# byronknoll/gmix

Hardware: AMD Instinct MI355X
Metric: mixer bits/sec (synthetic 256-input mixer streams, forward+update) (higher is better)
Workload: dtype f32; 1 GPU; configs[1]: synthetic 256-input 1-layer mixer (1 mixer, 2^16-row gate table), random logits, forward+update; n_inputs=256, mixers=1/0/0, streams_per_gpu=4096, total_bits=5486149632, parallelism=streams sharded over 1 GPU(s), no collective on the data path

## Files before the change

gmix_amd/csrc/gmx_capi.cpp:

```cpp
#include <hip/hip_runtime.h>
#include <math.h>
#include <stddef.h>
#include <stdio.h>
#include <stdlib.h>
#include <string.h>
#include <time.h>

#include <algorithm>
#include <atomic>
#include <map>
#include <new>
#include <string>
#include <vector>

#include "../../include/gmxmix.h"
#include "gmx_buildhash.h"
#include "gmx_internal.h"
#include "gmx_mailbox.h"
#include "gmx_ckpt.h"
#include "gmx_ind_ckpt.h"
#include "gmx_match.h"
#include "gmx_match_ckpt.h"
#include "gmx_ctx.h"
#include "gmx_ctx_ckpt.h"
// ... 220 lines not shown
  *dev_out = c.dev[k];
  return GMX_OK;
}
static int count_list_used(GmxCountList& c, hipStream_t st) {
  const int k = (int)((c.seq - 1u) % (unsigned)kStageSlots);
  HIPCHK(hipEventRecord(c.done[k], st));
  c.busy[k] = true;
  return GMX_OK;
}

struct gmx_group {
  int device = 0;
  int S = 0;
  GmxTopoDev topo;
  GmxTopoDev* topo_dev = nullptr;
  uint8_t* banks = nullptr;
  float* latch_out = nullptr;
  hipStream_t stream = nullptr;
  hipEvent_t ev0 = nullptr, ev1 = nullptr;
  unsigned lds_bytes = 0;
  std::vector<uint64_t> steps;
  std::vector<uint8_t> fwd_done;
  struct DecaySlot {
    float* dev = nullptr;
    uint32_t* idx_dev = nullptr;
    float* host = nullptr;
    uint32_t* idx_host = nullptr;
    size_t cap = 0;
    size_t idx_cap = 0;
    hipEvent_t done = nullptr;
    hipEvent_t ready = nullptr;
    bool busy = false;
    uint64_t* st_dev = nullptr;
    uint64_t* st_host = nullptr;
    uint32_t* amb_dev = nullptr;
    uint32_t* amb_host = nullptr;
    float* patch_host = nullptr;
    size_t st_cap = 0;
  } decay[kStageSlots];
  GmxCountList counts;
  hipStream_t copy_stream = nullptr;
  hipStream_t up_stream = nullptr, down_stream = nullptr;
  unsigned run_seq = 0;
  hipEvent_t tm0 = nullptr, tm1 = nullptr;
  gmx_batch* one = nullptr;
  std::vector<gmx_batch*> batches;
  std::vector<struct GmxSession*> sessions;
  std::vector<struct gmx_lockstep*> locksteps;
  bool banks_in_use_by_dead_kernel = false;
  bool use_sessions = true;
  bool mailbox_on_device = true;
  bool force_general = false;
  bool stock_exact = false;
  int stock_staged = -1;
  bool decay_on_host = false;
  bool stock_pairs = false;
  bool register_rows = false;
  int single_variant = 0;
  struct GmxCkptState* ckpt = nullptr;
};

struct gmx_batch {
  gmx_group* g = nullptr;
  int S = 0;
  uint64_t max_bits = 0;
  unsigned flags = 0;
  float* d_pred = nullptr;
  uint32_t* d_mask = nullptr;
  uint32_t* d_ctx = nullptr;
  uint8_t* d_bits = nullptr;
  float* d_p = nullptr;
  float* d_out = nullptr;
  float* d_last = nullptr;
  uint64_t* d_rng = nullptr;
  uint64_t* d_tcount = nullptr;
  float* d_pstate = nullptr;
  uint32_t* d_cstate = nullptr;
  float* h_pred = nullptr;
  uint32_t* h_mask = nullptr;
  uint32_t* h_ctx = nullptr;
  uint8_t* h_bits = nullptr;
  float* h_p = nullptr;
  float* h_out = nullptr;
  float* h_last = nullptr;
  GmxXfer x;
};

struct gmx_lockstep {
  gmx_group* g = nullptr;
  gmx_batch* b = nullptr;
  float* dec_host = nullptr;
  uint8_t* bits_host = nullptr;
  float* dec_dev = nullptr;
  uint32_t* idx_dev = nullptr;
  hipGraph_t g_predict = nullptr, g_learn = nullptr, g_step = nullptr;
  hipGraphExec_t x_predict = nullptr, x_learn = nullptr, x_step = nullptr;
  bool predicted = false;
  bool persistent = false, ps_running = false, ps_dead = false, ps_counted = false;
  hipStream_t ps_stream = nullptr;
  GmxLsDoor* door = nullptr;
  uint32_t* done = nullptr;
  uint32_t* blk_seen = nullptr;
  uint32_t* blk_replay = nullptr;
  uint32_t* relay = nullptr;
  float* live = nullptr;
  uint32_t seq = 0, word = 0, completed = 0;
// ... 458 lines not shown
  const bool wide = g->topo.l0 == 24 && g->topo.l1 == 8 && g->topo.n_skip == 1 && g->topo.has_final &&
                    ((g->topo.n == 256 && g->topo.mx[23].stride == 288) ||
                     (g->topo.n == 90 && g->topo.mx[23].stride == 128 && g->stock_pairs && !g->stock_exact)) &&
                    (mode & GMX_MODE_PREDICT) && !(mode & GMX_MODE_LATCH) && !g->force_general;
  return single ? GMX_K_SINGLE : wide ? GMX_K_WIDE : stock ? GMX_K_STOCK : GMX_K_BANK;
}

static int launch_run(gmx_group* g, gmx_batch* b, int s0, int rec0, int ns, uint64_t T,
                      unsigned mode, float* kernel_ms, const uint64_t* n_list = nullptr) {
  if (T == 0) return GMX_OK;
  for (gmx_lockstep* ls : g->locksteps) ls->predicted = false;
  gmx_group::DecaySlot* dec = nullptr;
  int rc = prepare_decay(g, s0, ns, T, (mode & GMX_MODE_LEARN) ? 1 : 0, &dec);
  if (rc) return rc;
  GmxRunArgs a;
  memset(&a, 0, sizeof a);
  a.banks = g->banks;
  a.pred = b->d_pred;
  a.mask = (b->flags & GMX_BATCH_MASK) ? b->d_mask : nullptr;
  a.ctx = b->d_ctx;
  a.bits = b->d_bits;
  a.decay = dec->dev;
  a.decay_idx = dec->idx_dev;
  a.p_out = b->d_p;
  a.out_all = (b->flags & GMX_BATCH_OUTPUTS) ? b->d_out : nullptr;
  a.out_last = (b->flags & GMX_BATCH_LAST_OUTPUTS) ? b->d_last : nullptr;
  a.latch_out = g->latch_out;
  a.rec_stride = b->max_bits;
  a.T = T;
  if (n_list) {
    int rcl = count_list_stage(g->counts, n_list, ns, g->stream, &a.T_list);
    if (rcl) return rcl;
  }
  a.mode = mode | (g->stock_exact ? GMX_MODE_EXACT : 0u);
  a.stream_base = s0;
  a.rec_base = rec0;
  a.n_streams = ns;
  {
    int rcx = xfer_before_run(b->x, g->stream);
    if (rcx) return rcx;
  }
  if (kernel_ms) HIPCHK(hipEventRecord(g->ev0, g->stream));
  const GmxKernelKind kind = kernel_for(g, mode);
  const bool single = kind == GMX_K_SINGLE, wide = kind == GMX_K_WIDE, stock = kind == GMX_K_STOCK;
  if (a.out_last && (single || wide)) return GMX_ERR_INVALID;
  if (kind == GMX_K_PAIR)
    HIPCHK(gmx_launch_pair_kernel(g->topo_dev, &a, ns, a.mask != nullptr, g->topo.n, g->topo.l0, g->topo.l1, g->stream));
  else if (single)
    HIPCHK(gmx_launch_single_kernel(g->topo_dev, &a, g->topo.n, g->single_variant, g->stream));
  else if (wide)
    HIPCHK(gmx_launch_wide_kernel(g->topo_dev, &a, ns, a.mask != nullptr, g->topo.n, g->stream));
  else if (stock)
    HIPCHK(gmx_launch_stock_kernel(g->topo_dev, &a, ns, GMX_STK_LDS_BYTES(g->topo.lds_misc),
                                   a.mask != nullptr, g->stock_staged, topo_tables_pow2(g->topo), g->stream));
  else
    HIPCHK(gmx_launch_bank_kernel(g->topo_dev, &a, ns, g->lds_bytes, a.mask != nullptr, g->topo.l0,
                                  g->topo.l1, g->topo.n_skip, g->topo.has_final,
                                  g->topo.mx[g->topo.l0 - 1].stride, g->stream));
  HIPCHK(hipEventRecord(dec->done, g->stream));
  dec->busy = true;
  if (n_list) {
    int rcl = count_list_used(g->counts, g->stream);
    if (rcl) return rcl;
  }
  {
    int rcn = batch_note_device_use(b);
    if (rcn) return rcn;
  }
  if (kernel_ms) {
    HIPCHK(hipEventRecord(g->ev1, g->stream));
    HIPCHK(hipEventSynchronize(g->ev1));
    HIPCHK(hipEventElapsedTime(kernel_ms, g->ev0, g->ev1));
  }
  if (mode & GMX_MODE_LEARN)
    for (int i = 0; i < ns; ++i) g->steps[s0 + i] += n_list ? n_list[i] : T;
  return GMX_OK;
}

static void batch_free(gmx_batch* b) {
  if (!b) return;
  if (b->g) {
    (void)hipSetDevice(b->g->device);
    if (b->g->stream) (void)hipStreamSynchronize(b->g->stream);
    if (b->g->up_stream) (void)hipStreamSynchronize(b->g->up_stream);
    if (b->g->down_stream) (void)hipStreamSynchronize(b->g->down_stream);
    auto& v = b->g->batches;
    v.erase(std::remove(v.begin(), v.end(), b), v.end());
  }
  void* dv[] = {b->d_pred, b->d_mask, b->d_ctx, b->d_bits, b->d_p, b->d_out, b->d_last,
                b->d_rng, b->d_tcount, b->d_pstate, b->d_cstate};
  for (void* p : dv)
    if (p) (void)hipFree(p);
  void* hv[] = {b->h_pred, b->h_mask, b->h_ctx, b->h_bits, b->h_p, b->h_out, b->h_last};
  for (void* p : hv)
    if (p) (void)hipHostFree(p);
  xfer_free(b->x);
  delete b;
}

static int batch_alloc(gmx_batch** out, gmx_group* g, int S, uint64_t max_bits, unsigned flags) {
  if (!out || !g || max_bits == 0) return GMX_ERR_INVALID;
  *out = nullptr;
  HIPCHK(hipSetDevice(g->device));
  gmx_batch* b = new (std::nothrow) gmx_batch();
  if (!b) return GMX_ERR_NOMEM;
  b->g = g;
  b->S = S;
// ... 504 lines not shown
  }
  HIPCHK(hipMalloc((void**)&tmp.dev, uniq.size() * T * sizeof(float)));
  int rc = decay_table_on_device(g, tmp, uniq, T);
  if (rc == GMX_OK) {
    if (n_unsettled) *n_unsettled = tmp.amb_host[0];
    std::vector<float> h(uniq.size() * T);
    hipError_t e = hipMemcpyAsync(h.data(), tmp.dev, h.size() * sizeof(float), hipMemcpyDeviceToHost, g->copy_stream);
    if (e == hipSuccess) e = hipStreamSynchronize(g->copy_stream);
    if (e != hipSuccess) rc = hip_fail(e, "gmx_debug_decay_table copy");
    else
      for (int u = 0; u < U; ++u) memcpy(out + (size_t)u * T, h.data() + (size_t)row[u] * T, T * sizeof(float));
  }
  void* dv[] = {tmp.dev, tmp.st_dev, tmp.amb_dev};
  for (void* p : dv)
    if (p) (void)hipFree(p);
  void* hv[] = {tmp.st_host, tmp.amb_host, tmp.patch_host};
  for (void* p : hv)
    if (p) (void)hipHostFree(p);
  return rc;
}

extern "C" int gmx_topology_register_rows_eligible(const gmx_topology* topo) {
  GmxTopoDev td;
  if (build_topology(topo, &td) != GMX_OK) return GMX_ERR_INVALID;
  return topo_register_rows_eligible(td) ? 1 : 0;
}

extern "C" int gmx_group_set_register_rows(gmx_group* g, int on) {
  if (!g || !topo_register_rows_eligible(g->topo)) return GMX_ERR_INVALID;
  g->register_rows = on != 0;
  return GMX_OK;
}

extern "C" int gmx_debug_force_general(gmx_group* g, int on) {
  if (!g) return GMX_ERR_INVALID;
  g->force_general = on != 0;
  return GMX_OK;
}

extern "C" int gmx_debug_kernel_kind(gmx_group* g, unsigned mode) {
  if (!g) return GMX_ERR_INVALID;
  const GmxKernelKind kind = kernel_for(g, mode);
  if (kind != GMX_K_BANK) return (int)kind;
  const GmxTopoDev& t = g->topo;
  return (int)kind + 4 * gmx_bank_kernel_build(t.l0, t.l1, t.n_skip, t.has_final, t.mx[t.l0 - 1].stride);
}

extern "C" int gmx_debug_stock_staged(gmx_group* g, int mode) {
  if (!g || mode < -1 || mode > 1) return GMX_ERR_INVALID;
  g->stock_staged = mode;
  return GMX_OK;
}

extern "C" int gmx_debug_stock_exact(gmx_group* g, int on) {
  if (!g) return GMX_ERR_INVALID;
  int rc = sessions_close(g, true);
  if (rc) return rc;
  g->stock_exact = on != 0;
  return GMX_OK;
}

extern "C" int gmx_debug_use_sessions(gmx_group* g, int on) {
  if (!g) return GMX_ERR_INVALID;
  int rc = sessions_close(g, true);
  if (rc) return rc;
  for (GmxSession* se : g->sessions)
    if (se && se->fwd_live) return GMX_ERR_STATE;
  g->use_sessions = on != 0;
  return GMX_OK;
}

extern "C" int gmx_debug_open_sessions(void) { return g_open_sessions.load(); }

extern "C" int gmx_debug_mailbox_on_device(gmx_group* g, int on, int stream, int* active) {
  if (!g) return GMX_ERR_INVALID;
  if (active) {
    GmxSession* se = (stream >= 0 && stream < (int)g->sessions.size()) ? g->sessions[stream] : nullptr;
    *active = (se && se->mc_on_device) ? 1 : 0;
  }
  if ((on != 0) == g->mailbox_on_device) return GMX_OK;
  int rc = sessions_close(g, true);
  if (rc) return rc;
  for (GmxSession* se : g->sessions)
    if (se && se->fwd_live) return GMX_ERR_STATE;
  sessions_free(g);
  g->mailbox_on_device = on != 0;
  return GMX_OK;
}

extern "C" int gmx_debug_per_bit_latency(gmx_group* g, int stream, int n, int ctx_hold, double* us_per_bit) {
  if (!g || n <= 0 || ctx_hold <= 0 || !us_per_bit) return GMX_ERR_INVALID;
  const GmxTopoDev& t = g->topo;
  std::vector<float> pred(t.n);
  std::vector<uint32_t> ctx(t.m, 0);
  uint64_t x = 0x9E3779B97F4A7C15ull;
  auto rnd = [&x]() { x ^= x << 13; x ^= x >> 7; x ^= x << 17; return x; };
  timespec a, b;
  clock_gettime(CLOCK_MONOTONIC, &a);
  for (int i = 0; i < n; ++i) {
    for (int k = 0; k < t.n; ++k) pred[k] = (float)((int64_t)(rnd() >> 40) - (1 << 23)) * (1.0f / (1 << 21));
    if (i % ctx_hold == 0)
      for (int k = 0; k < t.m; ++k) ctx[k] = (uint32_t)rnd();
    float p;
    int rc = gmx_bank_forward(g, stream, pred.data(), nullptr, -1, ctx.data(), &p, nullptr);
    if (rc) return rc;
    rc = gmx_bank_learn(g, stream, p > 0.5f ? 1 : 0);
// ... 461 lines not shown
```

gmix_amd/csrc/gmx_math.h:

```cpp
#ifndef GMX_MATH_H_
#define GMX_MATH_H_

#include <stdint.h>
#include <string.h>
#ifndef __cplusplus
#include <stdbool.h>
#endif

#if defined(__HIPCC__)
#include <hip/hip_runtime.h>
#define GMX_HD __host__ __device__ __forceinline__
#else
#define GMX_HD static inline
#endif

#if defined(__HIP_DEVICE_COMPILE__)
__device__ __constant__
#endif
static const uint64_t gmx_exp2f_tab[32] = {
    0x3ff0000000000000ull, 0x3fefd9b0d3158574ull, 0x3fefb5586cf9890full, 0x3fef9301d0125b51ull,
    0x3fef72b83c7d517bull, 0x3fef54873168b9aaull, 0x3fef387a6e756238ull, 0x3fef1e9df51fdee1ull,
    0x3fef06fe0a31b715ull, 0x3feef1a7373aa9cbull, 0x3feedea64c123422ull, 0x3feece086061892dull,
    0x3feebfdad5362a27ull, 0x3feeb42b569d4f82ull, 0x3feeab07dd485429ull, 0x3feea47eb03a5585ull,
    0x3feea09e667f3bcdull, 0x3fee9f75e8ec5f74ull, 0x3feea11473eb0187ull, 0x3feea589994cce13ull,
// ... 51 lines not shown
  float res = gmx_expf_main(x, tab);
  const bool big = abstop >= 0x42b;
  res = (big && x < -0x1.9d1d9ep6f) ? gmx_u2f(1u) : res;
  res = (big && x < -0x1.9fe368p6f) ? 0.0f : res;
  res = (big && x > 0x1.62e42ep6f) ? gmx_u2f(0x7f800000u) : res;
  res = (abstop >= 0x7f8) ? x + x : res;
  res = (ux == 0xff800000u) ? 0.0f : res;
  return res;
}

GMX_HD float gmx_expf(float x) { return gmx_expf_tab(x, gmx_exp2f_tab); }

GMX_HD float gmx_logistic_tab(float p, const uint64_t* tab) {
  return 1.0f / (1.0f + gmx_expf_tab(-p, tab));
}
GMX_HD float gmx_logistic(float p) { return gmx_logistic_tab(p, gmx_exp2f_tab); }

#if defined(__HIPCC__)
__device__ __forceinline__ bool gmx_wave_short_math(float p, uint64_t rs, uint64_t ms) {
  const uint32_t abstop = (gmx_f2u(p) >> 20) & 0x7ffu;
  return __ballot(abstop >= 0x428u || (uint32_t)((rs | ms) >> 32) != 0u) == 0;
}
__device__ __forceinline__ float gmx_logistic_short(float p, const uint64_t* tab) {
  const float d = 1.0f + gmx_expf_main(-p, tab);
  const float r0 = __builtin_amdgcn_rcpf(d);
  const float e0 = __builtin_fmaf(-d, r0, 1.0f);
  const float r1 = __builtin_fmaf(e0, r0, r0);
  const float e1 = __builtin_fmaf(-d, r1, 1.0f);
  const float q1 = __builtin_fmaf(e1, r1, r1);
  const float e2 = __builtin_fmaf(-d, q1, 1.0f);
  return __builtin_fmaf(e2, r1, q1);
}
__device__ __forceinline__ double gmx_row_age_short(uint64_t rs, uint64_t ms) {
  const double a = (double)(uint32_t)rs, b = (double)(uint32_t)ms;
  double r = __builtin_amdgcn_rcp(b);
  double e = __builtin_fma(-b, r, 1.0);
  r = __builtin_fma(r, e, r);
  e = __builtin_fma(-b, r, 1.0);
  r = __builtin_fma(r, e, r);
  const double q = a * r;
  e = __builtin_fma(-b, q, a);
  return __builtin_fma(e, r, q);
}
__device__ __forceinline__ float gmx_wave_logistic_and_age(float p, const uint64_t* tab, uint64_t rs, uint64_t ms,
                                                        double& age) {
  if (gmx_wave_short_math(p, rs, ms)) {
    age = gmx_row_age_short(rs, ms);
    return gmx_logistic_short(p, tab);
  }
  age = (double)rs / (double)ms;
  return gmx_logistic_tab(p, tab);
}

__device__ __forceinline__ float gmx_wave_logistic_and_age_hint(float p, const uint64_t* tab, uint64_t rs, uint64_t ms,
                                                             bool p_small, double& age) {
  if (p_small && __ballot((uint32_t)((rs | ms) >> 32) != 0u) == 0) {
    age = gmx_row_age_short(rs, ms);
    return gmx_logistic_short(p, tab);
  }
  age = (double)rs / (double)ms;
  return gmx_logistic_tab(p, tab);
}

__device__ __forceinline__ float gmx_wave_logistic(float p, const uint64_t* tab) {
  double unused;
  return gmx_wave_logistic_and_age(p, tab, 0, 1, unused);
}
__device__ __forceinline__ double gmx_wave_row_age(uint64_t rs, uint64_t ms) {
  if (__ballot((uint32_t)((rs | ms) >> 32) != 0u) == 0) return gmx_row_age_short(rs, ms);
  return (double)rs / (double)ms;
}

#endif

GMX_HD float gmx_clamp_prob(float prob) {
  const float eps = 0.0001f;
  return prob < eps ? eps : (prob > 1.0f - eps ? 1.0f - eps : prob);
}
GMX_HD float gmx_squash_clamp(float out) { return gmx_clamp_prob(gmx_logistic(out)); }

#if defined(__HIP_DEVICE_COMPILE__)
__device__ __constant__
#endif
static const uint64_t gmx_logf_tab[16][2] = {
    {0x3ff661ec79f8f3beull, 0xbfd57bf7808caadeull}, {0x3ff571ed4aaf883dull, 0xbfd2bef0a7c06ddbull},
    {0x3ff49539f0f010b0ull, 0xbfd01eae7f513a67ull}, {0x3ff3c995b0b80385ull, 0xbfcb31d8a68224e9ull},
    {0x3ff30d190c8864a5ull, 0xbfc6574f0ac07758ull}, {0x3ff25e227b0b8ea0ull, 0xbfc1aa2bc79c8100ull},
    {0x3ff1bb4a4a1a343full, 0xbfba4e76ce8c0e5eull}, {0x3ff12358f08ae5baull, 0xbfb1973c5a611cccull},
    {0x3ff0953f419900a7ull, 0xbfa252f438e10c1eull}, {0x3ff0000000000000ull, 0x0000000000000000ull},
    {0x3fee608cfd9a47acull, 0x3faaa5aa5df25984ull}, {0x3feca4b31f026aa0ull, 0x3fbc5e53aa362eb4ull},
    {0x3feb2036576afce6ull, 0x3fc526e57720db08ull}, {0x3fe9c2d163a1aa2dull, 0x3fcbc2860d224770ull},
    {0x3fe886e6037841edull, 0x3fd1058bc8a07ee1ull}, {0x3fe767dcf5534862ull, 0x3fd4043057b6ee09ull}};

GMX_HD float gmx_logf(float x) {
  const double kLn2 = 0x1.62e42fefa39efp-1;
  const double kA0 = -0x1.00ea348b88334p-2, kA1 = 0x1.5575b0be00b6ap-2, kA2 = -0x1.ffffef20a4123p-2;
  uint32_t ix = gmx_f2u(x);
  if (ix == 0x3f800000u) return 0.0f;
  if (ix - 0x00800000u >= 0x7f800000u - 0x00800000u) {
    if (ix * 2u == 0) return gmx_u2f(0xff800000u);
    if (ix == 0x7f800000u) return x;
    if ((ix & 0x80000000u) || ix * 2u >= 0xff000000u) return gmx_u2f(0x7fc00000u) + (x != x ? x : 0.0f);
    ix = gmx_f2u(x * 0x1p23f);
    ix -= 23u << 23;
  }
  const uint32_t tmp = ix - 0x3f330000u;
  const uint32_t i = (tmp >> 19) & 15u;
  const int32_t k = (int32_t)tmp >> 23;
  const uint32_t iz = ix - (tmp & 0xff800000u);
  const double invc = gmx_u2d(gmx_logf_tab[i][0]), logc = gmx_u2d(gmx_logf_tab[i][1]);
  const double z = (double)gmx_u2f(iz);
  const double r = gmx_fma(z, invc, -1.0);
  const double y0 = gmx_fma((double)k, kLn2, logc);
  const double r2 = r * r;
  double y = gmx_fma(kA1, r, kA2);
// ... 121 lines not shown
```

gmix_amd/csrc/gmx_stock.hip:

```cpp
#include <hip/hip_runtime.h>
#include <stdint.h>

#include "gmx_internal.h"
#include "gmx_math.h"
#include "gmx_stock_asm.inc"

typedef float gmx_f2 __attribute__((ext_vector_type(2)));
typedef float gmx_f4 __attribute__((ext_vector_type(4)));

#ifdef GMX_STK_PROF
__device__ unsigned long long gmx_stock_prof[16];
__device__ unsigned long long gmx_stock_prof_blk[4096][4];
#define STK_STAMP(i)                                                                  \
  do {                                                                                \
    if (blockIdx.x == 0 && threadIdx.x == 0) {                                        \
      const unsigned long long now_ = __builtin_amdgcn_s_memtime();                   \
      prof_lds[i] += (uint32_t)(now_ - tprev_);                                       \
      tprev_ = now_;                                                                  \
    }                                                                                 \
  } while (0)
#else
#define STK_STAMP(i)
#endif

namespace {

constexpr int kNPad = 92, kL0 = 24, kM = 33;
constexpr uint64_t kMaskL0 = (1ull << kL0) - 1, kMaskMx = (1ull << kM) - 1;

#define GMX_STOCK_KERNEL_ATTRS \
  __launch_bounds__(64) __attribute__((amdgpu_num_vgpr(GMX_STK_VGPR_LIMIT), amdgpu_num_sgpr(GMX_STK_SGPR_FIRST + 6)))

__device__ __forceinline__ uint32_t lds_addr(const void* p) {
  return (uint32_t)(uintptr_t)(__attribute__((address_space(3))) const void*)p;
}
__device__ __forceinline__ void dma16s(uint64_t sbase, uint32_t voff, uint32_t lds_byte_off) {
  uint32_t saved;
  asm volatile(
      "s_mov_b32 %0, m0\n\ts_mov_b32 m0, %3\n\ts_nop 0\n\t"
      "global_load_lds_dwordx4 %2, %1\n\ts_mov_b32 m0, %0"
      : "=&s"(saved)
      : "s"(sbase), "v"(voff), "s"(lds_byte_off)
      : "memory");
}
__device__ __forceinline__ void vld8(uint64_t& d, const uint64_t* p) {
  asm volatile("global_load_dwordx2 %0, %1, off" : "=a"(d) : "v"(p) : "memory");
}
__device__ __forceinline__ void vld4(uint32_t& d, const void* p) {
  asm volatile("global_load_dword %0, %1, off" : "=a"(d) : "v"(p) : "memory");
}
__device__ __forceinline__ void vld1(uint32_t& d, const uint8_t* p) {
  asm volatile("global_load_ubyte %0, %1, off" : "=a"(d) : "v"(p) : "memory");
}
__device__ __forceinline__ void vst8(void* p, uint64_t v) {
  asm volatile("global_store_dwordx2 %0, %1, off" : : "v"(p), "v"(v) : "memory");
}
__device__ __forceinline__ void vst4(void* p, float v) {
  asm volatile("global_store_dword %0, %1, off" : : "v"(p), "v"(v) : "memory");
}
template <int N>
__device__ __forceinline__ void vmcnt() {
  asm volatile("s_waitcnt vmcnt(%0)" : : "n"(N) : "memory");
}

__device__ __forceinline__ void stock_claim_registers() {
#pragma clang diagnostic push
#pragma clang diagnostic ignored "-Winline-asm"
  asm volatile("; gmx_stock_asm.inc uses v48..v255, a140..a255, s70..s101" ::: "v255", "a255", "s101");
#pragma clang diagnostic pop
  asm volatile(GMX_STK_ZERO);
}

constexpr uint32_t kPitchB = GMX_STK_ROW_PITCH;
constexpr uint32_t kImgB = kM * kPitchB;
constexpr int kSparseRows = 8;
__device__ __forceinline__ bool stock_sparse(uint64_t m) { return __builtin_popcountll(m) <= kSparseRows; }

template <bool STAGED>
__device__ __forceinline__ void stock_fetch_rows(const uint8_t* src, uint64_t nm, uint32_t img_in, uint32_t lane16) {
  uint64_t sv;
  if (!STAGED) {
    if (nm) asm volatile(GMX_STK_LOAD_A : [sv] "=&s"(sv) : [p] "v"(src), [mask] "s"(nm) : "memory");
    if (nm & kMaskL0)
      asm volatile(GMX_STK_LOAD_B : [sv] "=&s"(sv) : [p] "v"(src), [mask] "s"(nm & kMaskL0) : "memory");
    return;
  }
  if (!nm) return;
  const uint32_t plo = (uint32_t)(uint64_t)src, phi = (uint32_t)((uint64_t)src >> 32);
  if (!stock_sparse(nm)) {
    uint32_t sm0;
    asm volatile(GMX_STK_FETCH_ROWS
                 : [sv] "=&s"(sv), [sm0] "=&s"(sm0)
                 : [plo] "v"(plo), [phi] "v"(phi), [nm] "s"(nm), [img] "s"(img_in), [voff] "v"(lane16)
                 : "memory", "scc");
    return;
  }
  uint64_t m = nm;
  uint32_t sm0;
  asm volatile(GMX_STK_FETCH_SPARSE
               : [sv] "=&s"(sv), [sm0] "=&s"(sm0), [m] "+s"(m)
               : [plo] "v"(plo), [phi] "v"(phi), [img] "s"(img_in), [voff] "v"(lane16)
               : "memory", "scc");
}

typedef __attribute__((address_space(3))) float lds_float;
typedef __attribute__((address_space(3))) gmx_f4 lds_float4;
template <class F, class F4>
__device__ __forceinline__ void stock_mask_inputs_t(F* xin, uint32_t mword, int lane) {
  const uint32_t c = (uint32_t)lane * 4u;
  const uint32_t wd = (uint32_t)__builtin_amdgcn_ds_bpermute((int)(c >> 5) << 2, (int)mword);
  if (c < (uint32_t)kNPad) {
    gmx_f4 v = *(F4*)(xin + c);
    const uint32_t b = wd >> (c & 31u);
    v.x = (b & 1u) ? v.x : 0.f;
    v.y = (b & 2u) ? v.y : 0.f;
    v.z = (b & 4u) ? v.z : 0.f;
    v.w = (b & 8u) ? v.w : 0.f;
    *(F4*)(xin + c) = v;
  }
}
__device__ __forceinline__ void stock_mask_inputs(lds_float* xin, uint32_t mword, int lane) {
  stock_mask_inputs_t<lds_float, lds_float4>(xin, mword, lane);
}
__device__ __forceinline__ void stock_mask_inputs(float* xin, uint32_t mword, int lane) {
  const uint32_t c = (uint32_t)lane * 4u;
  const uint32_t wd = (uint32_t)__builtin_amdgcn_ds_bpermute((int)(c >> 5) << 2, (int)mword);
  if (c < (uint32_t)kNPad) {
    float4 v = *(float4*)(xin + c);
    const uint32_t b = wd >> (c & 31u);
    v.x = (b & 1u) ? v.x : 0.f;
    v.y = (b & 2u) ? v.y : 0.f;
    v.z = (b & 4u) ? v.z : 0.f;
    v.w = (b & 8u) ? v.w : 0.f;
    *(float4*)(xin + c) = v;
  }
}

__device__ __forceinline__ float stock_forward(uint32_t xaddr, float skip0, bool seen, bool is_mx, bool exact) {
  float acc, a1, t0, t1;
  bool redo = exact;
  if (!exact) {
    asm volatile(GMX_STK_FORWARD
                 : [acc] "=&v"(acc), [a1] "=&v"(a1), [t0] "=&v"(t0), [t1] "=&v"(t1)
                 : [xaddr] "v"(xaddr), [vskip] "v"(skip0)
                 : "vcc", "memory");
    redo = (__ballot(__builtin_amdgcn_classf(acc, 0x207)) & kMaskMx) != 0;
  }
  if (redo) {
    const uint64_t sm = __ballot(seen);
    uint64_t sv;
    asm volatile(GMX_STK_FORWARD_EXACT
                 : [acc] "=&v"(acc), [a1] "=&v"(a1), [t0] "=&v"(t0), [t1] "=&v"(t1), [sv] "=&s"(sv)
                 : [xaddr] "v"(xaddr), [vskip] "v"(skip0), [seenlo] "s"((uint32_t)sm),
                   [seenhi] "s"((uint32_t)(sm >> 32))
                 : "vcc", "memory");
  }
  return acc;
}

__device__ __forceinline__ float stock_forward_plain(uint32_t xaddr, float skip0, bool seen, bool& p_small) {
  float acc, a1, t0, t1;
  asm volatile(GMX_STK_FORWARD
               : [acc] "=&v"(acc), [a1] "=&v"(a1), [t0] "=&v"(t0), [t1] "=&v"(t1)
               : [xaddr] "v"(xaddr), [vskip] "v"(skip0)
               : "vcc", "memory");
  p_small = (__ballot((gmx_f2u(acc) & 0x7f800000u) > 0x42700000u) & kMaskMx) == 0;
  if (!p_small && (__ballot(__builtin_amdgcn_classf(acc, 0x207)) & kMaskMx) != 0) {
    const uint64_t sm = __ballot(seen);
    uint64_t sv;
    asm volatile(GMX_STK_FORWARD_EXACT
                 : [acc] "=&v"(acc), [a1] "=&v"(a1), [t0] "=&v"(t0), [t1] "=&v"(t1), [sv] "=&s"(sv)
                 : [xaddr] "v"(xaddr), [vskip] "v"(skip0), [seenlo] "s"((uint32_t)sm),
                   [seenhi] "s"((uint32_t)(sm >> 32))
                 : "vcc", "memory");
  }
  return acc;
}

__device__ __forceinline__ void stock_restore_forward(uint32_t xaddr, float acc) {
  asm volatile(GMX_STK_LOAD_X : : [xaddr] "v"(xaddr) : "memory");
  asm volatile(GMX_STK_OUTPUTS_TO_SGPRS : : [acc] "v"(acc));
}
__device__ __forceinline__ float stock_forward(const float* xin, float skip0, bool seen, bool is_mx, bool exact) {
  return stock_forward(lds_addr(xin), skip0, seen, is_mx, exact);
}

__device__ __forceinline__ void stock_update(float skip0, float upd, float scl) {
  const gmx_f2 up2 = {upd, upd};
  float t0, t1, ts;
  gmx_f2 p0, p1;
  uint64_t sv;
  asm volatile(GMX_STK_UPDATE
               : [t0] "=&v"(t0), [t1] "=&v"(t1), [ts] "=&v"(ts), [p0] "=&v"(p0), [p1] "=&v"(p1), [sv] "=&s"(sv)
               : [upd] "v"(upd), [up2] "v"(up2), [vskip] "v"(skip0)
               : "memory");
  if (__ballot(scl != 1.0f)) {
    const gmx_f2 sc2 = {scl, scl};
    asm volatile(GMX_STK_SHRINK : : [sc2] "v"(sc2));
  }
}

struct StockLane {
  uint64_t steps, max_steps, seen_cnt;
  uint64_t rs_w;
  uint32_t tag;
  bool dirty;
};

__device__ __forceinline__ float stock_learn_scalars(StockLane& st, double age, float dec, float lr, float pl,
                                                     uint32_t bit, bool is_mx, float& scl) {
  const double dd = (double)dec * (1.5 - age);
  const float decay = (float)dd;
  const float upd = decay * lr * (pl - (float)bit);
  const uint64_t rs_new = st.rs_w + 1;
  scl = ((rs_new & 1023u) == 0) ? (1.0f - 3.0e-6f) : 1.0f;
  if (is_mx) {
    ++st.steps;
    if (rs_new > st.max_steps) st.max_steps = rs_new;
    if (__ballot(st.rs_w == 0)) {
      if (st.rs_w == 0) ++st.seen_cnt;
    }
    st.rs_w = rs_new;
    st.dirty = true;
  }
  return upd;
}

template <bool STAGED>
__device__ __forceinline__ void stock_evict(const StockLane& st, bool ev, uint8_t* w_tab, uint8_t* rs_base,
                                            uint32_t rs_pitch, uint32_t row_bytes, bool folded, float* img_out_p,
                                            uint32_t img_out, int lane) {
  const uint64_t em = __ballot(ev);
  if (!em) return;
  uint8_t* dst = w_tab + (uint64_t)st.tag * row_bytes;
  uint64_t* const rs_dst = (uint64_t*)(rs_base + (uint64_t)st.tag * rs_pitch);
  uint64_t sv;
  if (!STAGED || stock_sparse(em)) {
    asm volatile(GMX_STK_STORE_A : [sv] "=&s"(sv) : [p] "v"(dst), [mask] "s"(em) : "memory");
    if (em & kMaskL0)
      asm volatile(GMX_STK_STORE_B : [sv] "=&s"(sv) : [p] "v"(dst), [mask] "s"(em & kMaskL0) : "memory");
    if (ev) vst8(rs_dst, st.rs_w);
    return;
  }
  if (ev) {
    if (folded) *(uint64_t*)((uint8_t*)img_out_p + (uint32_t)lane * kPitchB + row_bytes - 8u) = st.rs_w;
    else vst8(rs_dst, st.rs_w);
  }
  const uint32_t lrow = img_out + (uint32_t)lane * kPitchB;
  asm volatile(GMX_STK_TO_IMAGE_A : [sv] "=&s"(sv) : [l] "v"(lrow), [mask] "s"(em) : "memory");
  if (em & kMaskL0)
    asm volatile(GMX_STK_TO_IMAGE_B : [sv] "=&s"(sv) : [l] "v"(lrow), [mask] "s"(em & kMaskL0) : "memory");
  const uint32_t plo = (uint32_t)(uint64_t)dst, phi = (uint32_t)((uint64_t)dst >> 32);
  const uint32_t lane16 = (uint32_t)lane * 16u;
  asm volatile(GMX_STK_EVICT_ROWS
               : [sv] "=&s"(sv)
               : [plo] "v"(plo), [phi] "v"(phi), [em] "s"(em), [va] "v"(img_out + lane16), [voff] "v"(lane16)
               : "memory", "scc");
}

template <bool STAGED>
__device__ __forceinline__ uint64_t stock_adopt(uint64_t nm, bool need, uint32_t row_bytes, bool folded,
                                                const float* img_in_p, uint32_t img_in, int lane) {
  uint64_t sv;
  if (!STAGED) {
    asm volatile(GMX_STK_ADOPT_A : [sv] "=&s"(sv) : [mask] "s"(nm));
    if (nm & kMaskL0) asm volatile(GMX_STK_ADOPT_B : [sv] "=&s"(sv) : [mask] "s"(nm & kMaskL0));
    return 0;
  }
  const uint32_t lrow = img_in + (uint32_t)lane * kPitchB;
  asm volatile(GMX_STK_FROM_IMAGE_A : [sv] "=&s"(sv) : [l] "v"(lrow), [mask] "s"(nm) : "memory");
  if (nm & kMaskL0)
    asm volatile(GMX_STK_FROM_IMAGE_B : [sv] "=&s"(sv) : [l] "v"(lrow), [mask] "s"(nm & kMaskL0) : "memory");
  uint64_t rs = 0;
  if (need && folded) rs = *(const uint64_t*)((const uint8_t*)img_in_p + (uint32_t)lane * kPitchB + row_bytes - 8u);
  asm volatile("s_waitcnt lgkmcnt(0)" ::: "memory");
  return rs;
}

// ... 25 lines not shown
  if (lane < 32) s_tab[lane] = gmx_exp2f_tab[lane];
#ifdef GMX_STK_PROF
  uint32_t* const prof_lds = (uint32_t*)(lds + tp->lds_misc + 128);
  if (lane < 16) prof_lds[lane] = 0;
  unsigned long long tprev_ = __builtin_amdgcn_s_memtime();
  const unsigned long long blk_c0 = tprev_, blk_r0 = __builtin_amdgcn_s_memrealtime();
#endif

  const bool is_mx = lane < kM;
  const GmxMixerDev d = tp->mx[is_mx ? lane : 0];
  const int skip_idx = tp->skip_idx[0];
  const bool all_pow2 = PLAIN || __ballot((d.table_size & (d.table_size - 1u)) != 0) == 0;

  const uint64_t RS = a.rec_stride;
  const float* const pred_s = a.pred + (uint64_t)rec * RS * kNPad;
  const uint32_t* const mask_s = HAS_MASK ? a.mask + (uint64_t)rec * RS * MW : nullptr;
  const uint32_t* const ctx_s = a.ctx + (uint64_t)rec * RS * kM;
  const uint8_t* const bits_s = a.bits + (uint64_t)rec * RS;
  const float* const dec_s = a.decay + (uint64_t)a.decay_idx[blockIdx.x] * a.T;
  float* const p_s = a.p_out + (uint64_t)rec * RS;
  float* const oa_s = (!PLAIN && a.out_all) ? a.out_all + (uint64_t)rec * RS * kM : nullptr;
  float* const latch_s = a.latch_out + (uint64_t)s * kM;

  uint64_t* const scal = (uint64_t*)(bank + tp->scal_off) + 3 * lane;
  StockLane st = {0, 1, 0, 0, 0xffffffffu, false};
  if (is_mx) {
    st.steps = scal[0];
    st.max_steps = scal[1];
    st.seen_cnt = scal[2];
  }
  uint8_t* const rs_base = bank + d.rs_off;
  uint8_t* const w_tab = bank + d.w_off;
  const uint32_t row_bytes = d.stride * 4u;

  uint64_t nm_cur = 0;
  uint32_t x_cur = lds_addr(lds + tp->lds_in0);
  const uint32_t x_both = 2u * x_cur + in0_sz * 4u;
  uint32_t ctx_nn = is_mx ? ctx_s[lane] : 0;
  uint32_t row_n = 0, mask_n = ~0u, mask_c = ~0u, bit_n = 0, bit_c = 0;
  uint32_t dec_n = 0, dec_c = 0;
  uint64_t rs_ld = 0;
  bool need = false;
  const uint32_t lds_base = lds_addr(lds);
  const uint32_t lane16 = (uint32_t)lane * 16u;
  const uint32_t img_in = lds_base + (tp->lds_misc + 256u) * 4u, img_out = img_in + kImgB;
  float* const img_in_p = lds + tp->lds_misc + 256u;
  float* const img_out_p = img_in_p + kImgB / 4u;
  if (STAGED)
    for (uint32_t i = lane; i < kImgB / 16u; i += 64) ((float4*)img_out_p)[i] = float4{0.f, 0.f, 0.f, 0.f};
  const bool folded = PLAIN || d.rs_folded != 0;
  const bool rs_by_load = !(STAGED && folded);

  float acc_out = 0.f, pl_out = 0.f;
  auto prefetch = [&](const uint64_t t) __attribute__((always_inline)) {
    STK_STAMP(7);
    row_n = stock_row(ctx_nn, d.table_size, all_pow2);
    need = is_mx && row_n != st.tag;
    const uint8_t* src = w_tab + (uint64_t)row_n * row_bytes;
    nm_cur = __ballot(row_n != st.tag) & kMaskMx;
    stock_fetch_rows<STAGED>(src, nm_cur, img_in, lane16);
    if (need && rs_by_load) vld8(rs_ld, (const uint64_t*)(rs_base + (uint64_t)row_n * d.rs_pitch));
    {
      const uint64_t g = (uint64_t)(pred_s + t * (uint64_t)kNPad);
      if (lane16 < kNPad * 4u) dma16s(g, lane16, x_both - x_cur);
    }
    if (HAS_MASK) {
      mask_n = 0u;
      if (lane < MW) vld4(mask_n, mask_s + t * (uint64_t)MW + lane);
    }
    vld1(bit_n, bits_s + t);
    vld4(dec_n, dec_s + t);
    if (PLAIN) {
      vld4(ctx_nn, ctx_s + (t + 1) * (uint64_t)kM + (is_mx ? lane : kM - 1));
    } else {
      ctx_nn = 0u;
      if (is_mx && t + 1 < T) vld4(ctx_nn, ctx_s + (t + 1) * (uint64_t)kM + lane);
    }
    STK_STAMP(0);
  };
  auto compute = [&]() __attribute__((always_inline)) {
    lds_float* const xin = (lds_float*)x_cur;
    const bool seen = is_mx && st.rs_w != 0;
    const float skip0 = xin[skip_idx];
    if (HAS_MASK) stock_mask_inputs(xin, mask_c, lane);
    STK_STAMP(1);
    float acc;
    bool p_small = false;
    if (PLAIN) {
      acc = stock_forward_plain(x_cur, skip0, seen, p_small);
    } else if (do_predict) {
      acc = stock_forward(x_cur, skip0, seen, is_mx, exact);
    } else {
      acc = is_mx ? latch_s[lane] : 0.f;
      stock_restore_forward(x_cur, acc);
    }
    STK_STAMP(2);
    double age;
    const float pl = PLAIN ? gmx_wave_logistic_and_age_hint(acc, s_tab, st.rs_w, st.max_steps, p_small, age)
                           : gmx_wave_logistic_and_age(acc, s_tab, st.rs_w, st.max_steps, age);
    acc_out = acc;
    pl_out = pl;
    STK_STAMP(3);
    if (do_learn) {
      float scl;
      const float upd = stock_learn_scalars(st, age, __uint_as_float(dec_c), d.lr, pl, bit_c, PLAIN || is_mx, scl);
#ifdef GMX_STK_PROF
      asm volatile("" : : "v"(upd), "v"(scl));
#endif
      STK_STAMP(4);
      stock_update(skip0, upd, scl);
    }
    STK_STAMP(5);
  };
  auto commit = [&]() __attribute__((always_inline)) {
    vmcnt<0>();
    asm volatile("" : "+a"(rs_ld), "+a"(mask_n), "+a"(bit_n), "+a"(dec_n), "+a"(ctx_nn));
    STK_STAMP(6);
    if (nm_cur) {
      stock_evict<STAGED>(st, need && (PLAIN ? st.tag != 0xffffffffu : st.dirty), w_tab, rs_base, d.rs_pitch, row_bytes, folded, img_out_p, img_out, lane);
      const uint64_t rs_img = stock_adopt<STAGED>(nm_cur, need, row_bytes, folded, img_in_p, img_in, lane);
      if (need) {
        st.tag = row_n;
        st.rs_w = rs_by_load ? rs_ld : rs_img;
        st.dirty = false;
      }
    }
    x_cur = x_both - x_cur;
    mask_c = mask_n;
    bit_c = bit_n;
    dec_c = dec_n;
  };
  auto stores = [&](const uint64_t tc) __attribute__((always_inline)) {
    if (lane == kM - 1) vst4(p_s + tc, gmx_clamp_prob(pl_out));
    if (oa_s && is_mx) vst4(oa_s + tc * (uint64_t)kM + lane, acc_out);
    if (do_latch && is_mx) vst4(latch_s + lane, acc_out);
  };
  if (PLAIN) {
    prefetch(0);
    commit();
    for (uint64_t t = 1; t < T; ++t) {
      prefetch(t);
      compute();
      commit();
      stores(t - 1);
    }
    compute();
    stores(T - 1);
  } else {
    for (uint64_t t = 0; t <= T; ++t) {
      if (t < T) prefetch(t);
      if (t > 0) compute();
      if (t < T) commit();
      if (t > 0) stores(t - 1);
    }
  }
  if (a.out_last && is_mx) vst4(a.out_last + (uint64_t)rec * kM + lane, acc_out);
  vmcnt<0>();
  stock_evict<STAGED>(st, is_mx && (PLAIN ? st.tag != 0xffffffffu : st.dirty), w_tab, rs_base, d.rs_pitch, row_bytes, folded, img_out_p, img_out, lane);
  if (is_mx && do_learn) {
    scal[0] = st.steps;
    scal[1] = st.max_steps;
    scal[2] = st.seen_cnt;
  }
#ifdef GMX_STK_PROF
  if (blockIdx.x == 0 && lane < 16) atomicAdd(&gmx_stock_prof[lane], (unsigned long long)prof_lds[lane]);
  if (lane == 0 && blockIdx.x < 4096) {
    gmx_stock_prof_blk[blockIdx.x][0] = __builtin_amdgcn_s_memtime() - blk_c0;
    gmx_stock_prof_blk[blockIdx.x][1] = __builtin_amdgcn_s_memrealtime() - blk_r0;
    gmx_stock_prof_blk[blockIdx.x][2] = blk_r0;
    gmx_stock_prof_blk[blockIdx.x][3] = ((unsigned long long)__builtin_amdgcn_s_getreg(63508) << 32) | __builtin_amdgcn_s_getreg(63492);
  }
#endif
}

#ifdef GMX_STK_PROF
extern "C" int gmx_stock_prof_read(unsigned long long* out, int reset) {
  hipError_t e = hipMemcpyFromSymbol(out, HIP_SYMBOL(gmx_stock_prof), sizeof(unsigned long long) * 16);
  if (e == hipSuccess && reset) {
    unsigned long long z[16] = {0};
    e = hipMemcpyToSymbol(HIP_SYMBOL(gmx_stock_prof), z, sizeof z);
  }
  return (int)e;
}
extern "C" int gmx_stock_prof_blocks(unsigned long long* out, int n_blocks) {
  if (n_blocks > 4096) return -1;
  return (int)hipMemcpyFromSymbol(out, HIP_SYMBOL(gmx_stock_prof_blk), sizeof(unsigned long long) * 4 * n_blocks);
}
#endif

extern "C" hipError_t gmx_launch_stock_kernel(const GmxTopoDev* tp_dev, const GmxRunArgs* args,
                                              int n_streams, unsigned lds_bytes, int has_mask, int staged,
                                              int pow2_tables, hipStream_t stream) {
  (void)hipGetLastError();
  if (staged < 0) staged = n_streams >= 512 ? 1 : 0;
  const bool plain = pow2_tables && args->mode == (GMX_MODE_PREDICT | GMX_MODE_LEARN) && !args->out_all;
#define GMX_STK_LAUNCH(M, S, P) \
  hipLaunchKernelGGL((gmx_stock_kernel<M, S, P>), dim3(n_streams), dim3(64), lds_bytes, stream, tp_dev, *args)
  switch ((has_mask ? 4 : 0) | (staged ? 2 : 0) | (plain ? 1 : 0)) {
    case 7: GMX_STK_LAUNCH(true, true, true); break;
    case 6: GMX_STK_LAUNCH(true, true, false); break;
    case 5: GMX_STK_LAUNCH(true, false, true); break;
    case 4: GMX_STK_LAUNCH(true, false, false); break;
    case 3: GMX_STK_LAUNCH(false, true, true); break;
    case 2: GMX_STK_LAUNCH(false, true, false); break;
    case 1: GMX_STK_LAUNCH(false, false, true); break;
    default: GMX_STK_LAUNCH(false, false, false); break;
  }
#undef GMX_STK_LAUNCH
  return hipGetLastError();
}

// ... 430 lines not shown
```

Before: 1.837 billion bits/s.

## Specialize plain stock kernel step: scalar-base loads, periodic shrink, hoisted counter checks

Rewrites the per-step path of the plain stock mixer kernel. Loads and stores now use a scalar base plus a vector offset, and the LDS DMA sets m0 explicitly. A dedicated learn-scalars routine skips the general bookkeeping, with step and seen counting moved to adoption or kernel end. The weight shrink is applied only on a ballot over every 1024th row step instead of testing a per-step scale, and the large-counter check is cached across steps. A debug toggle to disable the plain path is also added. The aim is fewer VALU and SALU instructions and branches per bit, at the risk of small numeric or bookkeeping differences from the general path.

```diff
diff --git a/gmix_amd/csrc/gmx_capi.cpp b/gmix_amd/csrc/gmx_capi.cpp
--- a/gmix_amd/csrc/gmx_capi.cpp
+++ b/gmix_amd/csrc/gmx_capi.cpp
@@ -296,6 +296,7 @@
   bool mailbox_on_device = true;
   bool force_general = false;
   bool stock_exact = false;
+  bool stock_plain = true;
   int stock_staged = -1;
   bool decay_on_host = false;
   bool stock_pairs = false;
@@ -860,7 +861,7 @@
     HIPCHK(gmx_launch_wide_kernel(g->topo_dev, &a, ns, a.mask != nullptr, g->topo.n, g->stream));
   else if (stock)
     HIPCHK(gmx_launch_stock_kernel(g->topo_dev, &a, ns, GMX_STK_LDS_BYTES(g->topo.lds_misc),
-                                   a.mask != nullptr, g->stock_staged, topo_tables_pow2(g->topo), g->stream));
+                                   a.mask != nullptr, g->stock_staged, g->stock_plain && topo_tables_pow2(g->topo), g->stream));
   else
     HIPCHK(gmx_launch_bank_kernel(g->topo_dev, &a, ns, g->lds_bytes, a.mask != nullptr, g->topo.l0,
                                   g->topo.l1, g->topo.n_skip, g->topo.has_final,
@@ -1471,6 +1472,12 @@
   return GMX_OK;
 }
 
+extern "C" int gmx_debug_stock_plain(gmx_group* g, int on) {
+  if (!g) return GMX_ERR_INVALID;
+  g->stock_plain = on != 0;
+  return GMX_OK;
+}
+
 extern "C" int gmx_debug_stock_exact(gmx_group* g, int on) {
   if (!g) return GMX_ERR_INVALID;
   int rc = sessions_close(g, true);
diff --git a/gmix_amd/csrc/gmx_math.h b/gmix_amd/csrc/gmx_math.h
--- a/gmix_amd/csrc/gmx_math.h
+++ b/gmix_amd/csrc/gmx_math.h
@@ -127,15 +127,6 @@
   return gmx_logistic_tab(p, tab);
 }
 
-__device__ __forceinline__ float gmx_wave_logistic_and_age_hint(float p, const uint64_t* tab, uint64_t rs, uint64_t ms,
-                                                             bool p_small, double& age) {
-  if (p_small && __ballot((uint32_t)((rs | ms) >> 32) != 0u) == 0) {
-    age = gmx_row_age_short(rs, ms);
-    return gmx_logistic_short(p, tab);
-  }
-  age = (double)rs / (double)ms;
-  return gmx_logistic_tab(p, tab);
-}
 
 __device__ __forceinline__ float gmx_wave_logistic(float p, const uint64_t* tab) {
   double unused;
diff --git a/gmix_amd/csrc/gmx_stock.hip b/gmix_amd/csrc/gmx_stock.hip
--- a/gmix_amd/csrc/gmx_stock.hip
+++ b/gmix_amd/csrc/gmx_stock.hip
@@ -58,6 +58,24 @@
 __device__ __forceinline__ void vst4(void* p, float v) {
   asm volatile("global_store_dword %0, %1, off" : : "v"(p), "v"(v) : "memory");
 }
+__device__ __forceinline__ void vld4s(uint32_t& d, const void* sbase, uint32_t voff) {
+  asm volatile("global_load_dword %0, %1, %2" : "=a"(d) : "v"(voff), "s"(sbase) : "memory");
+}
+__device__ __forceinline__ void vld1s(uint32_t& d, const void* sbase, uint32_t voff) {
+  asm volatile("global_load_ubyte %0, %1, %2" : "=a"(d) : "v"(voff), "s"(sbase) : "memory");
+}
+__device__ __forceinline__ void vst4s_prev(const float* snext, uint32_t voff, float v) {
+  asm volatile("global_store_dword %0, %1, %2 offset:-4" : : "v"(voff), "v"(v), "s"(snext) : "memory");
+}
+__device__ __forceinline__ void dma16s_m0(uint64_t sbase, uint32_t voff, uint32_t lds_byte_off) {
+#pragma clang diagnostic push
+#pragma clang diagnostic ignored "-Winline-asm"
+  asm volatile("s_mov_b32 m0, %2\n\ts_nop 0\n\tglobal_load_lds_dwordx4 %1, %0"
+               :
+               : "s"(sbase), "v"(voff), "s"(lds_byte_off)
+               : "memory", "m0");
+#pragma clang diagnostic pop
+}
 template <int N>
 __device__ __forceinline__ void vmcnt() {
   asm volatile("s_waitcnt vmcnt(%0)" : : "n"(N) : "memory");
@@ -158,14 +176,18 @@
   return acc;
 }
 
-__device__ __forceinline__ float stock_forward_plain(uint32_t xaddr, float skip0, bool seen, bool& p_small) {
+__device__ __forceinline__ float stock_forward_plain(uint32_t xaddr, float skip0, uint64_t& wild) {
   float acc, a1, t0, t1;
   asm volatile(GMX_STK_FORWARD
                : [acc] "=&v"(acc), [a1] "=&v"(a1), [t0] "=&v"(t0), [t1] "=&v"(t1)
                : [xaddr] "v"(xaddr), [vskip] "v"(skip0)
                : "vcc", "memory");
-  p_small = (__ballot((gmx_f2u(acc) & 0x7f800000u) > 0x42700000u) & kMaskMx) == 0;
-  if (!p_small && (__ballot(__builtin_amdgcn_classf(acc, 0x207)) & kMaskMx) != 0) {
+  wild = __ballot((gmx_f2u(acc) & 0x7f800000u) > 0x42700000u) & kMaskMx;
+  return acc;
+}
+__device__ __forceinline__ float stock_forward_redo(float acc, uint32_t xaddr, float skip0, bool seen) {
+  if ((__ballot(__builtin_amdgcn_classf(acc, 0x207)) & kMaskMx) != 0) {
+    float a1, t0, t1;
     const uint64_t sm = __ballot(seen);
     uint64_t sv;
     asm volatile(GMX_STK_FORWARD_EXACT
@@ -185,7 +207,7 @@
   return stock_forward(lds_addr(xin), skip0, seen, is_mx, exact);
 }
 
-__device__ __forceinline__ void stock_update(float skip0, float upd, float scl) {
+__device__ __forceinline__ void stock_update_sweeps(float skip0, float upd) {
   const gmx_f2 up2 = {upd, upd};
   float t0, t1, ts;
   gmx_f2 p0, p1;
@@ -194,10 +216,14 @@
                : [t0] "=&v"(t0), [t1] "=&v"(t1), [ts] "=&v"(ts), [p0] "=&v"(p0), [p1] "=&v"(p1), [sv] "=&s"(sv)
                : [upd] "v"(upd), [up2] "v"(up2), [vskip] "v"(skip0)
                : "memory");
-  if (__ballot(scl != 1.0f)) {
-    const gmx_f2 sc2 = {scl, scl};
-    asm volatile(GMX_STK_SHRINK : : [sc2] "v"(sc2));
-  }
+}
+__device__ __forceinline__ void stock_shrink(float scl) {
+  const gmx_f2 sc2 = {scl, scl};
+  asm volatile(GMX_STK_SHRINK : : [sc2] "v"(sc2));
+}
+__device__ __forceinline__ void stock_update(float skip0, float upd, float scl) {
+  stock_update_sweeps(skip0, upd);
+  if (__ballot(scl != 1.0f)) stock_shrink(scl);
 }
 
 struct StockLane {
@@ -224,6 +250,21 @@
     st.dirty = true;
   }
   return upd;
+}
+
+__device__ __forceinline__ float stock_learn_scalars_plain(StockLane& st, double age, float dec, float lr, float pl,
+                                                           uint32_t bit) {
+  const double dd = (double)dec * (1.5 - age);
+  const float decay = (float)dd;
+  const float upd = decay * lr * (pl - (float)bit);
+  const uint64_t rs_new = st.rs_w + 1;
+  if (rs_new > st.max_steps) st.max_steps = rs_new;
+  st.rs_w = rs_new;
+  return upd;
+}
+
+__device__ __forceinline__ uint64_t stock_counters_big(const StockLane& st) {
+  return __ballot((uint32_t)((st.rs_w | st.max_steps) >> 32) != 0u);
 }
 
 template <bool STAGED>
@@ -355,6 +396,9 @@
   const bool rs_by_load = !(STAGED && folded);
 
   float acc_out = 0.f, pl_out = 0.f;
+  const uint32_t ctx_lane4 = 4u * (uint32_t)(is_mx ? lane : kM - 1);
+  const uint32_t* const ctx1_s = ctx_s + kM;
+  uint64_t cnt_big = PLAIN ? stock_counters_big(st) : 0;
   auto prefetch = [&](const uint64_t t) __attribute__((always_inline)) {
     STK_STAMP(7);
     row_n = stock_row(ctx_nn, d.table_size, all_pow2);
@@ -365,17 +409,22 @@
     if (need && rs_by_load) vld8(rs_ld, (const uint64_t*)(rs_base + (uint64_t)row_n * d.rs_pitch));
     {
       const uint64_t g = (uint64_t)(pred_s + t * (uint64_t)kNPad);
-      if (lane16 < kNPad * 4u) dma16s(g, lane16, x_both - x_cur);
+      if (lane16 < kNPad * 4u) {
+        if (PLAIN) dma16s_m0(g, lane16, x_both - x_cur);
+        else dma16s(g, lane16, x_both - x_cur);
+      }
     }
     if (HAS_MASK) {
       mask_n = 0u;
       if (lane < MW) vld4(mask_n, mask_s + t * (uint64_t)MW + lane);
     }
-    vld1(bit_n, bits_s + t);
-    vld4(dec_n, dec_s + t);
     if (PLAIN) {
-      vld4(ctx_nn, ctx_s + (t + 1) * (uint64_t)kM + (is_mx ? lane : kM - 1));
+      vld1s(bit_n, bits_s + t, 0u);
+      vld4s(dec_n, dec_s + t, 0u);
+      vld4s(ctx_nn, ctx1_s + t * (uint64_t)kM, ctx_lane4);
     } else {
+      vld1(bit_n, bits_s + t);
+      vld4(dec_n, dec_s + t);
       ctx_nn = 0u;
       if (is_mx && t + 1 < T) vld4(ctx_nn, ctx_s + (t + 1) * (uint64_t)kM + lane);
     }
@@ -388,10 +437,37 @@
     if (HAS_MASK) stock_mask_inputs(xin, mask_c, lane);
     STK_STAMP(1);
     float acc;
-    bool p_small = false;
     if (PLAIN) {
-      acc = stock_forward_plain(x_cur, skip0, seen, p_small);
-    } else if (do_predict) {
+      uint64_t wild;
+      acc = stock_forward_plain(x_cur, skip0, wild);
+      STK_STAMP(2);
+      double age;
+      float pl;
+      if (__builtin_expect((wild | cnt_big) == 0, 1)) {
+        age = gmx_row_age_short(st.rs_w, st.max_steps);
+        pl = gmx_logistic_short(acc, s_tab);
+      } else {
+        if (wild) acc = stock_forward_redo(acc, x_cur, skip0, seen);
+        age = (double)st.rs_w / (double)st.max_steps;
+        pl = gmx_logistic_tab(acc, s_tab);
+      }
+      acc_out = acc;
+      pl_out = pl;
+      STK_STAMP(3);
+      const float upd = stock_learn_scalars_plain(st, age, __uint_as_float(dec_c), d.lr, pl, bit_c);
+#ifdef GMX_STK_PROF
+      asm volatile("" : : "v"(upd));
+#endif
+      STK_STAMP(4);
+      stock_update_sweeps(skip0, upd);
+      if (__ballot(((uint32_t)st.rs_w & 1023u) == 0u)) {
+        stock_shrink(((uint32_t)st.rs_w & 1023u) == 0u ? (1.0f - 3.0e-6f) : 1.0f);
+        cnt_big = stock_counters_big(st);
+      }
+      STK_STAMP(5);
+      return;
+    }
+    if (do_predict) {
       acc = stock_forward(x_cur, skip0, seen, is_mx, exact);
     } else {
       acc = is_mx ? latch_s[lane] : 0.f;
@@ -399,14 +475,13 @@
     }
     STK_STAMP(2);
     double age;
-    const float pl = PLAIN ? gmx_wave_logistic_and_age_hint(acc, s_tab, st.rs_w, st.max_steps, p_small, age)
-                           : gmx_wave_logistic_and_age(acc, s_tab, st.rs_w, st.max_steps, age);
+    const float pl = gmx_wave_logistic_and_age(acc, s_tab, st.rs_w, st.max_steps, age);
     acc_out = acc;
     pl_out = pl;
     STK_STAMP(3);
     if (do_learn) {
       float scl;
-      const float upd = stock_learn_scalars(st, age, __uint_as_float(dec_c), d.lr, pl, bit_c, PLAIN || is_mx, scl);
+      const float upd = stock_learn_scalars(st, age, __uint_as_float(dec_c), d.lr, pl, bit_c, is_mx, scl);
 #ifdef GMX_STK_PROF
       asm volatile("" : : "v"(upd), "v"(scl));
 #endif
@@ -426,7 +501,9 @@
         st.tag = row_n;
         st.rs_w = rs_by_load ? rs_ld : rs_img;
         st.dirty = false;
-      }
+        if (PLAIN && st.rs_w == 0) ++st.seen_cnt;
+      }
+      if (PLAIN) cnt_big = stock_counters_big(st);
     }
     x_cur = x_both - x_cur;
     mask_c = mask_n;
@@ -434,6 +511,10 @@
     dec_c = dec_n;
   };
   auto stores = [&](const uint64_t tc) __attribute__((always_inline)) {
+    if (PLAIN) {
+      if (lane == kM - 1) vst4s_prev(p_s + tc + 1, 0u, gmx_clamp_prob(pl_out));
+      return;
+    }
     if (lane == kM - 1) vst4(p_s + tc, gmx_clamp_prob(pl_out));
     if (oa_s && is_mx) vst4(oa_s + tc * (uint64_t)kM + lane, acc_out);
     if (do_latch && is_mx) vst4(latch_s + lane, acc_out);
@@ -460,6 +541,7 @@
   if (a.out_last && is_mx) vst4(a.out_last + (uint64_t)rec * kM + lane, acc_out);
   vmcnt<0>();
   stock_evict<STAGED>(st, is_mx && (PLAIN ? st.tag != 0xffffffffu : st.dirty), w_tab, rs_base, d.rs_pitch, row_bytes, folded, img_out_p, img_out, lane);
+  if (PLAIN) st.steps += T;
   if (is_mx && do_learn) {
     scal[0] = st.steps;
     scal[1] = st.max_steps;
```

New measurement: 1.839 billion bits/s (median of 2 runs). No clear change (+0.1%).
